# chenchen235/SemStereo

Hardware: AMD Instinct MI355X
Metric: stereo pairs/sec, hot segment (gwc+concat volumes, 3-D hourglass stack, soft-argmax), 1024x1024 maxdisp=128 (higher is better)
Workload: dtype f32; 1 GPU; BASELINE.json configs[1]: 1024x1024, maxdisp=128, batch=1/GPU x 1 GPU(s); features [B,128,H/4,W/4]+[B,256,H/8,W/8] -> disparity; input_sets_rotated=3, execution=steps round-robin on 6 HIP streams (PairPipeline); bit-identical to one stream, conv_engine=f16x3, hip_graph=False

## Files before the change

### semstereo_amd/csrc/common.cpp

```cpp
#include "common.h"

#include <stdlib.h>
#include <string.h>

#include <atomic>
#include <mutex>
#include <unordered_map>

namespace {
thread_local char g_last_error[256] = "";

int env_int(const char* name) {
    const char* v = getenv(name);
    if (v == nullptr) return -1;
    return ((v[0] >= '0' && v[0] <= '9') || (v[0] == '-' && v[1] >= '0' && v[1] <= '9')) ? atoi(v) : 1;
}

ss::Tuning read_tuning() {
    ss::Tuning t;
    t.conv_tile = env_int("SS_CONV_TILE");
    t.conv_s2_mt1 = env_int("SS_CONV_S2_MT1");
    t.gwc_stream = env_int("SS_GWC_STREAM");
    t.warp_stream = env_int("SS_WARP_STREAM");
    t.warp_vec4 = env_int("SS_WARP_VEC") == 4 ? 1 : 0;
    t.warp_generic = env_int("SS_WARP_GENERIC");
    t.deconv_split = env_int("SS_DECONV_SPLIT");
    t.deconv_groups = env_int("SS_DECONV_GROUPS");
    if (t.deconv_groups > 2) t.deconv_groups = -1;
    t.deconv_stream = env_int("SS_DECONV_STREAM");
    t.wgrad_coop = env_int("SS_WGRAD_COOP");
    t.fill_hint = env_int("SS_FILL_HINT");
    return t;
}

ss::Tuning g_tuning[2];
std::atomic<int> g_tuning_slot{-1};
std::mutex g_mutex;
std::atomic<int> g_fill_hint{1};
constexpr int kMaxFillHint = 64;
std::unordered_map<unsigned long long, int> g_lds_set;
}

namespace ss {
void note_hip_error(hipError_t e) {
    const char* s = hipGetErrorString(e);
    strncpy(g_last_error, s ? s : "unknown hip error", sizeof(g_last_error) - 1);
    g_last_error[sizeof(g_last_error) - 1] = 0;
}

const Tuning& tuning() {
    int slot = g_tuning_slot.load(std::memory_order_acquire);
    if (slot < 0) {
        std::lock_guard<std::mutex> lock(g_mutex);
        slot = g_tuning_slot.load(std::memory_order_relaxed);
        if (slot < 0) {
            g_tuning[0] = read_tuning();
            g_tuning_slot.store(slot = 0, std::memory_order_release);
        }
    }
    return g_tuning[slot];
}

int fill_hint() {
    const int env = tuning().fill_hint;
    const int h = env >= 1 ? env : g_fill_hint.load(std::memory_order_relaxed);
    return h < 1 ? 1 : (h > kMaxFillHint ? kMaxFillHint : h);
}

int ensure_dynamic_lds(const void* kernel, int bytes) {
    if (bytes <= 64 * 1024) return SS_OK;
    int dev = 0;
    if (hipGetDevice(&dev) != hipSuccess) dev = 0;
    const unsigned long long key = (unsigned long long)reinterpret_cast<uintptr_t>(kernel) * 64ull + (unsigned)dev;
    std::lock_guard<std::mutex> lock(g_mutex);
    auto it = g_lds_set.find(key);
    if (it != g_lds_set.end() && it->second >= bytes) return SS_OK;
    hipError_t e = hipFuncSetAttribute(kernel, hipFuncAttributeMaxDynamicSharedMemorySize, bytes);
    if (e != hipSuccess) {
        note_hip_error(e);
        return SS_ERR_LAUNCH;
    }
    g_lds_set[key] = bytes;
    return SS_OK;
}

int resident_workgroups(const void* kernel, int block, int lds_bytes) {
    static std::unordered_map<unsigned long long, int> cache;
    int dev = 0;
    if (hipGetDevice(&dev) != hipSuccess) dev = 0;
    const unsigned long long key = (unsigned long long)reinterpret_cast<uintptr_t>(kernel) * 64ull + (unsigned)dev;
    std::lock_guard<std::mutex> lock(g_mutex);
    auto it = cache.find(key);
    if (it != cache.end()) return it->second;
    int per_cu = 0, cus = 0;
    if (hipOccupancyMaxActiveBlocksPerMultiprocessor(&per_cu, kernel, block, (size_t)lds_bytes) != hipSuccess || per_cu < 1) per_cu = 2;
    if (hipDeviceGetAttribute(&cus, hipDeviceAttributeMultiprocessorCount, dev) != hipSuccess || cus < 1) cus = 256;
    (void)hipGetLastError();
    return cache[key] = per_cu * cus;
}
}

extern "C" int ss_reload_tuning(void) {
    std::lock_guard<std::mutex> lock(g_mutex);
    const int cur = g_tuning_slot.load(std::memory_order_relaxed);
    const int nxt = cur == 0 ? 1 : 0;
    g_tuning[nxt] = read_tuning();
    g_tuning_slot.store(nxt, std::memory_order_release);
    return SS_OK;
}

extern "C" int ss_set_fill_hint(int pairs_in_flight) {
    return g_fill_hint.exchange(pairs_in_flight < 1 ? 1 : (pairs_in_flight > kMaxFillHint ? kMaxFillHint : pairs_in_flight), std::memory_order_relaxed);
}

extern "C" int ss_get_fill_hint(void) { return ss::fill_hint(); }

extern "C" int ss_abi_version(void) { return 20; }

extern "C" const char* ss_status_string(int status) {
    switch (status) {
        case SS_OK: return "ok";
        case SS_ERR_INVALID: return "invalid argument (null pointer, non-positive size, or C % groups != 0)";
        case SS_ERR_UNSUPPORTED: return "shape not supported by the gfx950 kernels";
        case SS_ERR_LAUNCH: return "kernel launch failed (see ss_last_hip_error)";
        default: return "unknown status";
    }
}

extern "C" const char* ss_last_hip_error(void) { return g_last_error; }
```

### semstereo_amd/csrc/common.h

```cpp
#pragma once
#include <hip/hip_runtime.h>
#include <stdint.h>

#include "../../include/semstereo_hip.h"

namespace ss {

constexpr int kWave = 64;

void note_hip_error(hipError_t e);

inline int check_launch() {
    hipError_t e = hipGetLastError();
    if (e != hipSuccess) {
        note_hip_error(e);
        return SS_ERR_LAUNCH;
    }
    return SS_OK;
}

inline hipStream_t as_stream(ss_stream_t s) { return reinterpret_cast<hipStream_t>(s); }

struct Tuning {
    int conv_tile;
    int conv_s2_mt1;
    int gwc_stream;
    int warp_stream;
    int warp_vec4;
    int warp_generic;
    int deconv_split;
    int deconv_groups;
    int deconv_stream;
    int wgrad_coop;
    int fill_hint;
};
const Tuning& tuning();
int fill_hint();

int ensure_dynamic_lds(const void* kernel, int bytes);
int resident_workgroups(const void* kernel, int block, int lds_bytes);

__host__ __device__ inline int ceil_div(int a, int b) { return (a + b - 1) / b; }

inline int range_halo(int dmin, int ndisp) {
    const int a = -dmin, b = dmin + ndisp - 1;
    const int m = a > b ? a : b;
    return m <= 0 ? 0 : (m + 3) / 4 * 4;
}
__host__ __device__ inline long long ceil_div_ll(long long a, long long b) { return (a + b - 1) / b; }

struct Packed {
    long long terms, total;
};
inline float* scales_of(void* wsplit, const Packed& p) { return reinterpret_cast<float*>(static_cast<char*>(wsplit) + p.terms); }
inline const float* scales_of(const void* wsplit, const Packed& p) {
    return reinterpret_cast<const float*>(static_cast<const char*>(wsplit) + p.terms);
}

__device__ __forceinline__ float mul_rn(float a, float b) {
#pragma clang fp contract(off)
    return a * b;
}
__device__ __forceinline__ float add_rn(float a, float b) {
#pragma clang fp contract(off)
    return a + b;
}
__device__ __forceinline__ float sub_rn(float a, float b) {
#pragma clang fp contract(off)
    return a - b;
}
__device__ __forceinline__ float exp_fast(float x) {
    const float L = 1.44269502162933349609375f, Llo = 1.925962991126617e-8f;
    const float t = __fmul_rn(x, L);
    const float e = __fmaf_rn(x, L, -t) + x * Llo;
    const float p = __builtin_amdgcn_exp2f(t);
    return __fmaf_rn(p, e * 0.693147180559945f, p);
}

__device__ __forceinline__ void lds_add(float* p, float v) {
    typedef float __attribute__((address_space(3))) * lds_ptr_t;
    __hip_atomic_fetch_add((lds_ptr_t)(p), v, __ATOMIC_RELAXED, __HIP_MEMORY_SCOPE_WORKGROUP);
}

typedef volatile float __attribute__((address_space(3))) * lds_vf_t;
typedef volatile int __attribute__((address_space(3))) * lds_vi_t;
__device__ __forceinline__ void lds_owned_add(int* tag, unsigned k, bool take, float* row, float v) {
    const int me = (int)__lane_id();
    bool pending = take;
    while (__builtin_amdgcn_ballot_w64(pending) != 0) {
        if (pending) {
            ((lds_vi_t)tag)[k] = me;
            const int won = ((lds_vi_t)tag)[k];
            const float a = ((lds_vf_t)row)[k];
            if (won == me) {
                ((lds_vf_t)row)[k] = a + v;
                pending = false;
            }
        }
    }
}
__device__ __forceinline__ void lds_owned_add2(int* tag, unsigned k, bool take, float* row_a, float va, float* row_b, float vb, bool two) {
    const int me = (int)__lane_id();
    bool pending = take;
    while (__builtin_amdgcn_ballot_w64(pending) != 0) {
        if (pending) {
            ((lds_vi_t)tag)[k] = me;
            const int won = ((lds_vi_t)tag)[k];
            const float a = ((lds_vf_t)row_a)[k];
            const float b = two ? ((lds_vf_t)row_b)[k] : 0.f;
            if (won == me) {
                ((lds_vf_t)row_a)[k] = a + va;
                if (two) ((lds_vf_t)row_b)[k] = b + vb;
                pending = false;
            }
        }
    }
}
template <int N>
__device__ __forceinline__ void lds_owned_addn(int* tag, unsigned k, bool take, float* row0, int stride, const float (&v)[N], int nlive) {
    const int me = (int)__lane_id();
    bool pending = take;
    if (nlive == N) {
        while (__builtin_amdgcn_ballot_w64(pending) != 0) {
            if (pending) {
                ((lds_vi_t)tag)[k] = me;
                const int won = ((lds_vi_t)tag)[k];
                float a[N];
#pragma unroll
                for (int n = 0; n < N; ++n) a[n] = ((lds_vf_t)(row0 + n * stride))[k];
                if (won == me) {
#pragma unroll
                    for (int n = 0; n < N; ++n) ((lds_vf_t)(row0 + n * stride))[k] = a[n] + v[n];
                    pending = false;
                }
            }
        }
        return;
    }
    while (__builtin_amdgcn_ballot_w64(pending) != 0) {
        if (pending) {
            ((lds_vi_t)tag)[k] = me;
            const int won = ((lds_vi_t)tag)[k];
            float a[N];
#pragma unroll
            for (int n = 0; n < N; ++n) a[n] = (n < nlive) ? ((lds_vf_t)(row0 + n * stride))[k] : 0.f;
            if (won == me) {
#pragma unroll
                for (int n = 0; n < N; ++n)
                    if (n < nlive) ((lds_vf_t)(row0 + n * stride))[k] = a[n] + v[n];
                pending = false;
            }
        }
    }
}
__device__ __forceinline__ float lds_ld(const float* p) { return *(const float __attribute__((address_space(3)))*)p; }
__device__ __forceinline__ float lds_get(const float* p) { return *(lds_vf_t)p; }
__device__ __forceinline__ void lds_put(float* p, float v) { *(lds_vf_t)p = v; }

typedef float lds_v4f __attribute__((ext_vector_type(4)));
__device__ __forceinline__ void lds_read16(const float* p, float* dst) {
    typedef const volatile lds_v4f __attribute__((address_space(3))) * ptr_t;
    const lds_v4f q = *(ptr_t)(p);
    dst[0] = q.x; dst[1] = q.y; dst[2] = q.z; dst[3] = q.w;
}

}

int ss_softmax_regress_split_launch(const float* logits, float* prob, float* disp, float* var, int B, int dmin, int ndisp,
                                    int H, int W, hipStream_t st);

#define SS_REQUIRE(cond)              \
    do {                                \
        if (!(cond)) return SS_ERR_INVALID; \
    } while (0)
```

### semstereo_amd/csrc/window_attention.hip

```cpp
#include <algorithm>

#include "common.h"
#include "split_f16.h"

namespace {


constexpr int HD = 8;
constexpr int HG = 4;

template <int T, int C>
struct ACfg {
    static constexpr int NTL = (T + 31) / 32;
    static constexpr int TP = NTL * 32;
    static constexpr int XS = C * TP;
    static constexpr int QKV = 3 * 32 * TP;
    static constexpr int YG = 32 * TP;
    static constexpr int FLAGS = TP;
    static constexpr int WL = C * 96;
    static constexpr size_t LDS_BYTES = (size_t)(XS + QKV + YG + FLAGS + WL) * 4;
};

template <int T, int C>
__device__ __forceinline__ void stage_window_tokens(float* __restrict__ xs, const float* __restrict__ xb, int tid, int wd, int wh,
                                                    int ww, int H, int W, int bd, int bh, int bw, size_t plane, size_t vol) {
    using A = ACfg<T, C>;
    if (bw == 4 && (W & 3) == 0 && ((reinterpret_cast<uintptr_t>(xb) & 15) == 0)) {
        constexpr int NQ = C * (A::TP / 4) / 256;
        static_assert(C * (A::TP / 4) % 256 == 0, "whole batches");
#pragma unroll
        for (int i = 0; i < NQ; ++i) {
            const int e = tid + 256 * i;
            const int tq = e % (A::TP / 4), c = e / (A::TP / 4);
            const int ih = tq % bh, id = tq / bh;
            const int gh = wh * bh + ih, gd = wd * bd + id, gw = ww * 4;
            const bool ok = gh < H && gw < W;
            const float4 q = *reinterpret_cast<const float4*>(xb + (size_t)c * vol + (size_t)gd * plane +
                                                              (size_t)min(gh, H - 1) * W + min(gw, W - 4));
            *reinterpret_cast<float4*>(&xs[e * 4]) = ok ? q : make_float4(0.f, 0.f, 0.f, 0.f);
        }
    } else {
        for (int e = tid; e < C * A::TP; e += 256) {
            const int t = e % A::TP, c = e / A::TP;
            float v = 0.f;
            if (t < T) {
                const int iw = t % bw, ih = (t / bw) % bh, id = t / (bw * bh);
                const int gw = ww * bw + iw, gh = wh * bh + ih, gd = wd * bd + id;
                if (gh < H && gw < W) v = xb[(size_t)c * vol + (size_t)gd * plane + (size_t)gh * W + gw];
            }
            xs[e] = v;
        }
    }
}

template <int T, int C>
__global__ __launch_bounds__(256) void window_attention_kernel(
    const float* __restrict__ x, const float* __restrict__ wqkv_t, const float* __restrict__ bqkv,
    const float* __restrict__ wout_t, const float* __restrict__ bout, float* __restrict__ out, int D, int H, int W,
    int bd, int bh, int bw, int nwh, int nww, int use_mask) {
    using A = ACfg<T, C>;
    extern __shared__ __attribute__((aligned(16))) float lds[];
    float* xs = lds;
    float* qkv = xs + A::XS;
    float* yg = qkv + A::QKV;
    float* flag = yg + A::YG;
    float* wl = flag + A::FLAGS;

    const int tid = threadIdx.x, lane = tid & 63, wave = tid >> 6;
    const int l31 = lane & 31, half = lane >> 5;
    int wi = blockIdx.x;
    const int ww = wi % nww; wi /= nww;
    const int wh = wi % nwh; wi /= nwh;
    const int wd = wi;
    const int b = blockIdx.y;
    const size_t plane = (size_t)H * W, vol = (size_t)D * plane;
    const float* xb = x + (size_t)b * C * vol;

    stage_window_tokens<T, C>(xs, xb, tid, wd, wh, ww, H, W, bd, bh, bw, plane, vol);
    for (int t = tid; t < A::TP; t += 256) {
        float f = 0.f;
        if (t < T) {
            const int iw = t % bw, ih = (t / bw) % bh;
            f = ((wh * bh + ih >= H) || (ww * bw + iw >= W)) ? 1.f : 0.f;
        }
        flag[t] = f;
    }
    __syncthreads();

    static_assert(C == 128, "4 waves x 32 output channels");
    f32x16 oacc[A::NTL];
#pragma unroll
    for (int n = 0; n < A::NTL; ++n)
#pragma unroll
        for (int r = 0; r < 16; ++r) oacc[n][r] = 0.f;

    const float scale = 0.35355339059327379f;
    constexpr int NGROUPS = C / (HG * HD);

    constexpr int NWQ = C * 24 / 256;
    float4 wreg[NWQ];
    const float* wsrc[NWQ];
#pragma unroll
    for (int i = 0; i < NWQ; ++i) {
        const int e = tid + 256 * i;
        wsrc[i] = wqkv_t + (size_t)(e / 24) * 3 * C + ((e % 24) / 8) * C + ((e % 24) % 8) * 4;
        wreg[i] = *reinterpret_cast<const float4*>(wsrc[i]);
    }

    for (int g = 0; g < NGROUPS; ++g) {
#pragma unroll
        for (int i = 0; i < NWQ; ++i) {
            const int e = tid + 256 * i;
            *reinterpret_cast<float4*>(&wl[(e / 24) * 96 + (e % 24) * 4]) = wreg[i];
        }
        __syncthreads();
        if (g + 1 < NGROUPS) {
#pragma unroll
            for (int i = 0; i < NWQ; ++i) wreg[i] = *reinterpret_cast<const float4*>(wsrc[i] + (g + 1) * 32);
        }
        for (int u = wave; u < 3 * A::NTL; u += 4) {
            const int mt = u / A::NTL, nt = u % A::NTL;
            const int f0 = mt * C + g * 32;
            f32x16 acc;
#pragma unroll
            for (int r = 0; r < 16; ++r) acc[r] = 0.f;
            const float* ap = wl + half * 96 + mt * 32 + l31;
            const float* bp = xs + half * A::TP + nt * 32 + l31;
#pragma unroll 8
            for (int kk = 0; kk < C; kk += 2)
                acc = __builtin_amdgcn_mfma_f32_32x32x2f32(ap[kk * 96], bp[kk * A::TP], acc, 0, 0, 0);
#pragma unroll
            for (int r = 0; r < 16; ++r) {
                const int row = (r & 3) + 8 * (r >> 2) + 4 * half;
                qkv[(mt * 32 + row) * A::TP + nt * 32 + l31] = ss::add_rn(acc[r], bqkv[f0 + row]);
            }
        }
        __syncthreads();

        static_assert(A::TP == T, "windows of 64 / 96 tokens are whole 32-token tiles");
        for (int u = wave; u < HG * A::NTL; u += 4) {
            const int hh = u / A::NTL, qt = u % A::NTL;
            f32x16 st[A::NTL];
#pragma unroll
            for (int kt = 0; kt < A::NTL; ++kt) {
#pragma unroll
                for (int r = 0; r < 16; ++r) st[kt][r] = 0.f;
#pragma unroll
                for (int sd = 0; sd < HD / 2; ++sd)
                    st[kt] = __builtin_amdgcn_mfma_f32_32x32x2f32(
                        qkv[(32 + hh * HD + 2 * sd + half) * A::TP + kt * 32 + l31],
                        qkv[(hh * HD + 2 * sd + half) * A::TP + qt * 32 + l31],
                        st[kt], 0, 0, 0);
            }
            const float fq = flag[qt * 32 + l31];
            float mx = -INFINITY;
#pragma unroll
            for (int kt = 0; kt < A::NTL; ++kt)
#pragma unroll
                for (int r = 0; r < 16; ++r) {
                    float d = ss::mul_rn(st[kt][r], scale);
                    if (use_mask && flag[kt * 32 + (r & 3) + 8 * (r >> 2) + 4 * half] != fq) d = ss::add_rn(d, -1000.0f);
                    st[kt][r] = d;
                    mx = fmaxf(mx, d);
                }
            mx = fmaxf(mx, __shfl_xor(mx, 32));
            float sum = 0.f;
#pragma unroll
            for (int kt = 0; kt < A::NTL; ++kt)
#pragma unroll
                for (int r = 0; r < 16; ++r) { st[kt][r] = ss::exp_fast(st[kt][r] - mx); sum = ss::add_rn(sum, st[kt][r]); }
            sum = ss::add_rn(sum, __shfl_xor(sum, 32));
            const float rsum = 1.0f / sum;
            f32x16 ot;
#pragma unroll
            for (int r = 0; r < 16; ++r) ot[r] = 0.f;
            const float* vrow = qkv + (64 + hh * HD + (l31 & 7)) * A::TP + 4 * half;
#pragma unroll
            for (int kt = 0; kt < A::NTL; ++kt)
#pragma unroll
                for (int r = 0; r < 16; ++r) {
                    const float vv = (l31 < HD) ? vrow[kt * 32 + (r & 3) + 8 * (r >> 2)] : 0.f;
                    ot = __builtin_amdgcn_mfma_f32_32x32x2f32(vv, ss::mul_rn(st[kt][r], rsum), ot, 0, 0, 0);
                }
#pragma unroll
            for (int r = 0; r < 4; ++r) yg[(hh * HD + 4 * half + r) * A::TP + qt * 32 + l31] = ot[r];
        }
        __syncthreads();

        {
            const float* ap = wout_t + (size_t)(g * 32 + half) * C + wave * 32 + l31;
            const float* bp = yg + half * A::TP + l31;
#pragma unroll
            for (int kk = 0; kk < 32; kk += 2) {
                const float a = ap[(size_t)kk * C];
#pragma unroll
                for (int n = 0; n < A::NTL; ++n)
                    oacc[n] = __builtin_amdgcn_mfma_f32_32x32x2f32(a, bp[kk * A::TP + n * 32], oacc[n], 0, 0, 0);
            }
        }
        __syncthreads();
    }

    float* ob = out + (size_t)b * C * vol;
#pragma unroll
    for (int n = 0; n < A::NTL; ++n) {
        const int t = n * 32 + l31;
        if (t >= T) continue;
        const int iw = t % bw, ih = (t / bw) % bh, id = t / (bw * bh);
        const int gw = ww * bw + iw, gh = wh * bh + ih, gd = wd * bd + id;
        if (gh >= H || gw >= W) continue;
        const size_t pos = (size_t)gd * plane + (size_t)gh * W + gw;
#pragma unroll
        for (int r = 0; r < 16; ++r) {
            const int co = wave * 32 + (r & 3) + 8 * (r >> 2) + 4 * half;
            ob[(size_t)co * vol + pos] = ss::add_rn(oacc[n][r], bout[co]);
        }
    }
}

template <int T, int C>
__device__ __forceinline__ void attend_head_group(float* __restrict__ qkv, const float* __restrict__ flag, const unsigned (&vmax_w)[4],
                                                  float* __restrict__ y, int b, int g, int wd, int wh, int ww, int D, int H, int W,
                                                  int bd, int bh, int bw, int use_mask);

template <int T, int C>
__global__ __launch_bounds__(256) void window_attention_core(const float* __restrict__ qkv_in, const float* __restrict__ bqkv,
                                                              float* __restrict__ y, int D, int H, int W, int bd, int bh,
                                                              int bw, int nwh, int nww, int use_mask) {
    using A = ACfg<T, C>;
    static_assert(A::TP == T, "windows of 64 / 96 tokens are whole 32-token tiles");
    __shared__ __attribute__((aligned(16))) float qkv[3 * 32 * A::TP];
    __shared__ float flag[A::TP];
    const int tid = threadIdx.x, lane = tid & 63, wave = tid >> 6;
    constexpr int NGROUPS = C / (HG * HD);
    int wi = blockIdx.x;
    const int g = wi % NGROUPS; wi /= NGROUPS;
    const int ww = wi % nww; wi /= nww;
    const int wh = wi % nwh; wi /= nwh;
    const int wd = wi;
    const int b = blockIdx.y;
    const size_t plane = (size_t)H * W, vol = (size_t)D * plane;
    const float* qb = qkv_in + (size_t)b * 3 * C * vol;

    __shared__ unsigned vmax_w[4];
    float vm = 0.f;
    if (bw == 4 && (W & 3) == 0 && ((reinterpret_cast<uintptr_t>(qkv_in) & 15) == 0)) {
        constexpr int NQ = 96 * (A::TP / 4) / 256;
        static_assert(96 * (A::TP / 4) % 256 == 0, "whole batches");
#pragma unroll
        for (int i = 0; i < NQ; ++i) {
            const int e = tid + 256 * i;
            const int tq = e % (A::TP / 4), row = e / (A::TP / 4);
            const int f = (row >> 5) * C + g * 32 + (row & 31);
            const int ih = tq % bh, id = tq / bh;
            const int gh = wh * bh + ih, gd = wd * bd + id, gw = ww * 4;
            const bool ok = gh < H && gw < W;
            const float4 q = *reinterpret_cast<const float4*>(qb + (size_t)f * vol + (size_t)gd * plane +
                                                              (size_t)min(gh, H - 1) * W + min(gw, W - 4));
            const float bf = bqkv[f];
            const float4 v4 = ok ? q : make_float4(bf, bf, bf, bf);
            *reinterpret_cast<float4*>(&qkv[e * 4]) = v4;
            if (row >= 64) vm = fmaxf(vm, fmaxf(fmaxf(fabsf(v4.x), fabsf(v4.y)), fmaxf(fabsf(v4.z), fabsf(v4.w))));
        }
    } else {
        for (int e = tid; e < 96 * A::TP; e += 256) {
            const int t = e % A::TP, row = e / A::TP;
            const int f = (row >> 5) * C + g * 32 + (row & 31);
            const int iw = t % bw, ih = (t / bw) % bh, id = t / (bw * bh);
            const int gw = ww * bw + iw, gh = wh * bh + ih, gd = wd * bd + id;
            const float v1 = (gh < H && gw < W) ? qb[(size_t)f * vol + (size_t)gd * plane + (size_t)gh * W + gw] : bqkv[f];
            qkv[e] = v1;
            if (row >= 64) vm = fmaxf(vm, fabsf(v1));
        }
    }
    {
        const unsigned wm = wave_max_bits(__float_as_uint(vm));
        if (lane == 0) vmax_w[wave] = wm;
    }
    for (int t = tid; t < A::TP; t += 256) {
        const int iw = t % bw, ih = (t / bw) % bh;
        flag[t] = ((wh * bh + ih >= H) || (ww * bw + iw >= W)) ? 1.f : 0.f;
    }
    __syncthreads();
    attend_head_group<T, C>(qkv, flag, vmax_w, y, b, g, wd, wh, ww, D, H, W, bd, bh, bw, use_mask);
}

template <int T, int C>
__device__ __forceinline__ void attend_head_group(float* __restrict__ qkv, const float* __restrict__ flag, const unsigned (&vmax_w)[4],
                                                  float* __restrict__ y, int b, int g, int wd, int wh, int ww, int D, int H, int W,
                                                  int bd, int bh, int bw, int use_mask) {
    using A = ACfg<T, C>;
    const int tid = threadIdx.x, lane = tid & 63, wave = tid >> 6;
    const int l31 = lane & 31, half = lane >> 5;
    const size_t plane = (size_t)H * W, vol = (size_t)D * plane;
    const float scale = 0.35355339059327379f;
    const int e_v = workgroup_exponent(vmax_w);
    const float v_scale = scale_for(e_v);
    const float pv_unscale = unscale_for(e_v) * (1.0f / 16384.0f);
    for (int wk = tid; wk < 32 * (A::TP / 16); wk += 256) {
        float* base = qkv + (64 + wk / (A::TP / 16)) * A::TP + (wk % (A::TP / 16)) * 16;
        float f[16];
#pragma unroll
        for (int k4 = 0; k4 < 4; ++k4) ss::lds_read16(base + 4 * k4, &f[4 * k4]);
#pragma unroll
        for (int h = 0; h < 2; ++h) {
            unsigned hi[4], lo[4];
#pragma unroll
            for (int j = 0; j < 4; ++j) {
                const int t0 = (j < 2) ? 4 * h + 2 * j : 8 + 4 * h + 2 * (j - 2);
                split2_pk_f16(f[t0] * v_scale, f[t0 + 1] * v_scale, hi[j], lo[j]);
            }
            *reinterpret_cast<uint4*>(base + 8 * h) = make_uint4(hi[0], hi[1], hi[2], hi[3]);
            *reinterpret_cast<uint4*>(base + 8 * h + 4) = make_uint4(lo[0], lo[1], lo[2], lo[3]);
        }
    }
    __syncthreads();
    float* yb = y + (size_t)b * C * vol;
    for (int u = wave; u < HG * A::NTL; u += 4) {
        const int hh = u / A::NTL, qt = u % A::NTL;
        f32x16 st[A::NTL];
#pragma unroll
        for (int kt = 0; kt < A::NTL; ++kt) {
#pragma unroll
            for (int r = 0; r < 16; ++r) st[kt][r] = 0.f;
#pragma unroll
            for (int sd = 0; sd < HD / 2; ++sd)
                st[kt] = __builtin_amdgcn_mfma_f32_32x32x2f32(
                    qkv[(32 + hh * HD + 2 * sd + half) * A::TP + kt * 32 + l31],
                    qkv[(hh * HD + 2 * sd + half) * A::TP + qt * 32 + l31],
                    st[kt], 0, 0, 0);
        }
        const float fq = flag[qt * 32 + l31];
        float mx = -INFINITY;
#pragma unroll
        for (int kt = 0; kt < A::NTL; ++kt)
#pragma unroll
            for (int r = 0; r < 16; ++r) {
                float d = ss::mul_rn(st[kt][r], scale);
                if (use_mask && flag[kt * 32 + (r & 3) + 8 * (r >> 2) + 4 * half] != fq) d = ss::add_rn(d, -1000.0f);
                st[kt][r] = d;
                mx = fmaxf(mx, d);
            }
        mx = fmaxf(mx, __shfl_xor(mx, 32));
        float sum = 0.f;
#pragma unroll
        for (int kt = 0; kt < A::NTL; ++kt)
#pragma unroll
            for (int r = 0; r < 16; ++r) { st[kt][r] = ss::exp_fast(st[kt][r] - mx); sum = ss::add_rn(sum, st[kt][r]); }
        sum = ss::add_rn(sum, __shfl_xor(sum, 32));
        const float rsum = 1.0f / sum;
        f32x16 ot;
#pragma unroll
        for (int r = 0; r < 16; ++r) ot[r] = 0.f;
        const float* vrow = qkv + (64 + hh * HD + (l31 & 7)) * A::TP + 8 * half;
        const float ps = rsum * 16384.0f;
#pragma unroll
        for (int kt = 0; kt < A::NTL; ++kt)
#pragma unroll
            for (int s8 = 0; s8 < 2; ++s8) {
                float vh[4], vl[4];
                ss::lds_read16(vrow + kt * 32 + 16 * s8, vh);
                ss::lds_read16(vrow + kt * 32 + 16 * s8 + 4, vl);
                unsigned bh_[4], bl_[4];
#pragma unroll
                for (int j = 0; j < 4; ++j)
                    split2_pk_f16(st[kt][8 * s8 + 2 * j] * ps, st[kt][8 * s8 + 2 * j + 1] * ps, bh_[j], bl_[j]);
                const f16x8 a_hi = __builtin_bit_cast(f16x8, make_float4(vh[0], vh[1], vh[2], vh[3]));
                const f16x8 a_lo = __builtin_bit_cast(f16x8, make_float4(vl[0], vl[1], vl[2], vl[3]));
                const f16x8 b_hi = __builtin_bit_cast(f16x8, make_uint4(bh_[0], bh_[1], bh_[2], bh_[3]));
                const f16x8 b_lo = __builtin_bit_cast(f16x8, make_uint4(bl_[0], bl_[1], bl_[2], bl_[3]));
                ot = __builtin_amdgcn_mfma_f32_32x32x16_f16(a_hi, b_lo, ot, 0, 0, 0);
                ot = __builtin_amdgcn_mfma_f32_32x32x16_f16(a_lo, b_hi, ot, 0, 0, 0);
                ot = __builtin_amdgcn_mfma_f32_32x32x16_f16(a_hi, b_hi, ot, 0, 0, 0);
            }
#pragma unroll
        for (int r = 0; r < 4; ++r) ot[r] *= pv_unscale;
        const int t = qt * 32 + l31;
        const int iw = t % bw, ih = (t / bw) % bh, id = t / (bw * bh);
        const int gw = ww * bw + iw, gh = wh * bh + ih, gd = wd * bd + id;
        if (gh < H && gw < W) {
            const size_t pos = (size_t)gd * plane + (size_t)gh * W + gw;
#pragma unroll
            for (int r = 0; r < 4; ++r) yb[(size_t)(g * 32 + hh * HD + 4 * half + r) * vol + pos] = ot[r];
        }
    }
}

template <int T, int C, int NTERMS, int KH>
__global__ __launch_bounds__(256, KH == 2 ? 4 : 3) void window_attention_proj(const float* __restrict__ x, const uint4* __restrict__ wsplit,
                                                              const float* __restrict__ bqkv, float* __restrict__ y, int D, int H,
                                                              int W, int bd, int bh, int bw, int nwh, int nww, int use_mask) {
    using A = ACfg<T, C>;
    static_assert(A::TP == T && C % (32 * KH) == 0 && (KH == 1 || KH == 2), "whole 32-token tiles, whole K-steps per stage");
    constexpr int NC = (NTERMS == 6) ? 3 : 2;
    constexpr int KS = C / 16;
    constexpr int CH = C / KH;
    __shared__ __attribute__((aligned(16))) float buf[(CH > 96 ? CH : 96) * A::TP];
    __shared__ float flag[A::TP];
    __shared__ unsigned vmax_w[4];
    const int tid = threadIdx.x, lane = tid & 63, wave = tid >> 6;
    const int l31 = lane & 31, half = lane >> 5;
    constexpr int NGROUPS = C / (HG * HD);
    int wi = blockIdx.x;
    const int g = wi % NGROUPS; wi /= NGROUPS;
    const int ww = wi % nww; wi /= nww;
    const int wh = wi % nwh; wi /= nwh;
    const int wd = wi;
    const int b = blockIdx.y;
    const size_t plane = (size_t)H * W, vol = (size_t)D * plane;

    for (int t = tid; t < A::TP; t += 256) {
        const int iw = t % bw, ih = (t / bw) % bh;
        flag[t] = ((wh * bh + ih >= H) || (ww * bw + iw >= W)) ? 1.f : 0.f;
    }
    constexpr int NU = (3 * A::NTL + 3) / 4;
    f32x16 acc[NU];
#pragma unroll
    for (int i = 0; i < NU; ++i)
#pragma unroll
        for (int r = 0; r < 16; ++r) acc[i][r] = 0.f;
#pragma unroll
    for (int kh = 0; kh < KH; ++kh) {
        if (kh > 0) __syncthreads();
        stage_window_tokens<T, CH>(buf, x + ((size_t)b * C + kh * CH) * vol, tid, wd, wh, ww, H, W, bd, bh, bw, plane, vol);
        __syncthreads();
#pragma unroll
        for (int i = 0; i < NU; ++i) {
            const int u = wave + 4 * i;
            if (u >= 3 * A::NTL) continue;
            const int mt = u / A::NTL, nt = u % A::NTL;
            const uint4* ap = wsplit + (size_t)(mt * (C / 32) + g) * KS * 3 * 64 + half * 32 + l31;
            const float* bp = buf + 8 * half * A::TP + nt * 32 + l31;
#pragma unroll
            for (int k = 0; k < KS / KH; ++k) {
                const int ks = kh * (KS / KH) + k;
                bf16x8 a[NC];
#pragma unroll
                for (int c = 0; c < NC; ++c) a[c] = __builtin_bit_cast(bf16x8, ap[(ks * 3 + c) * 64]);
                unsigned bh_[4], bm_[4], bl_[4];
#pragma unroll
                for (int j = 0; j < 4; ++j)
                    split3_pk(bp[(k * 16 + 2 * j) * A::TP], bp[(k * 16 + 2 * j + 1) * A::TP], bh_[j], bm_[j], bl_[j]);
                const bf16x8 h8 = __builtin_bit_cast(bf16x8, make_uint4(bh_[0], bh_[1], bh_[2], bh_[3]));
                const bf16x8 m8 = __builtin_bit_cast(bf16x8, make_uint4(bm_[0], bm_[1], bm_[2], bm_[3]));
                if (NTERMS == 6) {
                    const bf16x8 l8 = __builtin_bit_cast(bf16x8, make_uint4(bl_[0], bl_[1], bl_[2], bl_[3]));
                    acc[i] = __builtin_amdgcn_mfma_f32_32x32x16_bf16(a[1], m8, acc[i], 0, 0, 0);
                    acc[i] = __builtin_amdgcn_mfma_f32_32x32x16_bf16(a[0], l8, acc[i], 0, 0, 0);
                    acc[i] = __builtin_amdgcn_mfma_f32_32x32x16_bf16(a[NC - 1], h8, acc[i], 0, 0, 0);
                }
                acc[i] = __builtin_amdgcn_mfma_f32_32x32x16_bf16(a[0], m8, acc[i], 0, 0, 0);
                acc[i] = __builtin_amdgcn_mfma_f32_32x32x16_bf16(a[1], h8, acc[i], 0, 0, 0);
                acc[i] = __builtin_amdgcn_mfma_f32_32x32x16_bf16(a[0], h8, acc[i], 0, 0, 0);
            }
        }
    }
    float bias[NU][16];
#pragma unroll
    for (int i = 0; i < NU; ++i) {
        const int u = wave + 4 * i;
        if (u >= 3 * A::NTL) continue;
#pragma unroll
        for (int r = 0; r < 16; ++r) bias[i][r] = bqkv[(u / A::NTL) * C + g * 32 + (r & 3) + 8 * (r >> 2) + 4 * half];
    }
    __syncthreads();
    float vm = 0.f;
#pragma unroll
    for (int i = 0; i < NU; ++i) {
        const int u = wave + 4 * i;
        if (u >= 3 * A::NTL) continue;
        const int mt = u / A::NTL, nt = u % A::NTL;
#pragma unroll
        for (int r = 0; r < 16; ++r) {
            const float v = ss::add_rn(acc[i][r], bias[i][r]);
            buf[(mt * 32 + (r & 3) + 8 * (r >> 2) + 4 * half) * A::TP + nt * 32 + l31] = v;
            if (mt == 2) vm = fmaxf(vm, fabsf(v));
        }
    }
    {
        const unsigned wm = wave_max_bits(__float_as_uint(vm));
        if (lane == 0) vmax_w[wave] = wm;
    }
    __syncthreads();
    attend_head_group<T, C>(buf, flag, vmax_w, y, b, g, wd, wh, ww, D, H, W, bd, bh, bw, use_mask);
}

#ifndef SS_ATTN_PROJ_KH96
#define SS_ATTN_PROJ_KH96 2
#endif
template <int T, int NTERMS>
int launch_attn_proj(const float* x, const void* wsplit, const float* bqkv, float* y, int B, int D, int H, int W, int bd, int bh,
                     int bw, hipStream_t st) {
    const int nwd = D / bd, nwh = ss::ceil_div(H, bh), nww = ss::ceil_div(W, bw);
    const int use_mask = (H % bh != 0) && (W % bw != 0);
    const long long nblk = (long long)nwd * nwh * nww * (128 / (HG * HD));
    if (nblk > 0x7fffffffLL || B > 65535) return SS_ERR_UNSUPPORTED;
    hipLaunchKernelGGL((window_attention_proj<T, 128, NTERMS, T == 96 ? SS_ATTN_PROJ_KH96 : 1>), dim3((unsigned)nblk, B), dim3(256), 0, st, x,
                       reinterpret_cast<const uint4*>(wsplit), bqkv, y, D, H, W, bd, bh, bw, nwh, nww, use_mask);
    return ss::check_launch();
}

template <int T>
int launch_attn_core(const float* qkv, const float* bqkv, float* y, int B, int D, int H, int W, int bd, int bh, int bw,
                     hipStream_t st) {
    const int nwd = D / bd, nwh = ss::ceil_div(H, bh), nww = ss::ceil_div(W, bw);
    const int use_mask = (H % bh != 0) && (W % bw != 0);
    const long long nblk = (long long)nwd * nwh * nww * (128 / (HG * HD));
    if (nblk > 0x7fffffffLL || B > 65535) return SS_ERR_UNSUPPORTED;
    hipLaunchKernelGGL((window_attention_core<T, 128>), dim3((unsigned)nblk, B), dim3(256), 0, st, qkv, bqkv, y, D, H, W, bd,
                       bh, bw, nwh, nww, use_mask);
    return ss::check_launch();
}

template <int T>
int launch_attn(const float* x, const float* wqkv_t, const float* bqkv, const float* wout_t, const float* bout,
                float* out, int B, int D, int H, int W, int bd, int bh, int bw, hipStream_t st) {
    using A = ACfg<T, 128>;
    const int nwd = D / bd, nwh = ss::ceil_div(H, bh), nww = ss::ceil_div(W, bw);
    const int use_mask = (H % bh != 0) && (W % bw != 0);
    auto kern = window_attention_kernel<T, 128>;
    if (A::LDS_BYTES > 64 * 1024) {
        if (ss::ensure_dynamic_lds(reinterpret_cast<const void*>(kern), (int)A::LDS_BYTES) != SS_OK) return SS_ERR_LAUNCH;
    }
    const long long nwin = (long long)nwd * nwh * nww;
    if (nwin > 0x7fffffffLL || B > 65535) return SS_ERR_UNSUPPORTED;
    hipLaunchKernelGGL(kern, dim3((unsigned)nwin, B), dim3(256), A::LDS_BYTES, st, x, wqkv_t, bqkv, wout_t, bout, out, D,
                       H, W, bd, bh, bw, nwh, nww, use_mask);
    return ss::check_launch();
}

}

extern "C" int ss_window_attention_fwd(const float* x, const float* wqkv_t, const float* bqkv, const float* wout_t,
                                       const float* bout, float* out, int B, int C, int D, int H, int W, int heads,
                                       int bd, int bh, int bw, ss_stream_t stream) {
    SS_REQUIRE(x && wqkv_t && bqkv && wout_t && bout && out);
    SS_REQUIRE(B > 0 && C > 0 && D > 0 && H > 0 && W > 0 && heads > 0 && bd > 0 && bh > 0 && bw > 0);
    SS_REQUIRE(D % bd == 0);
    if (C != 128 || heads != 16) return SS_ERR_UNSUPPORTED;
    const int T = bd * bh * bw;
    hipStream_t st = ss::as_stream(stream);
    if (T == 64) return launch_attn<64>(x, wqkv_t, bqkv, wout_t, bout, out, B, D, H, W, bd, bh, bw, st);
    if (T == 96) return launch_attn<96>(x, wqkv_t, bqkv, wout_t, bout, out, B, D, H, W, bd, bh, bw, st);
    return SS_ERR_UNSUPPORTED;
}

extern "C" int ss_window_attention_core_fwd(const float* qkv, const float* bqkv, float* y, int B, int C, int D, int H,
                                            int W, int heads, int bd, int bh, int bw, ss_stream_t stream) {
    SS_REQUIRE(qkv && bqkv && y);
    SS_REQUIRE(B > 0 && C > 0 && D > 0 && H > 0 && W > 0 && heads > 0 && bd > 0 && bh > 0 && bw > 0);
    SS_REQUIRE(D % bd == 0);
    if (C != 128 || heads != 16) return SS_ERR_UNSUPPORTED;
    const int T = bd * bh * bw;
    hipStream_t st = ss::as_stream(stream);
    if (T == 64) return launch_attn_core<64>(qkv, bqkv, y, B, D, H, W, bd, bh, bw, st);
    if (T == 96) return launch_attn_core<96>(qkv, bqkv, y, B, D, H, W, bd, bh, bw, st);
    return SS_ERR_UNSUPPORTED;
}

extern "C" int ss_window_attention_proj_fwd(const float* x, const void* wqkv_split, const float* bqkv, float* y, int B, int C,
                                            int D, int H, int W, int heads, int bd, int bh, int bw, int nterms,
                                            ss_stream_t stream) {
    SS_REQUIRE(x && wqkv_split && bqkv && y);
    SS_REQUIRE(B > 0 && C > 0 && D > 0 && H > 0 && W > 0 && heads > 0 && bd > 0 && bh > 0 && bw > 0);
    SS_REQUIRE(D % bd == 0 && (nterms == 3 || nterms == 6));
    SS_REQUIRE((reinterpret_cast<uintptr_t>(wqkv_split) & 15) == 0);
    if (C != 128 || heads != 16) return SS_ERR_UNSUPPORTED;
    const int T = bd * bh * bw;
    hipStream_t st = ss::as_stream(stream);
#define SS_AP(TV)                                                                                                     \
    if (T == TV)                                                                                                      \
        return nterms == 6 ? launch_attn_proj<TV, 6>(x, wqkv_split, bqkv, y, B, D, H, W, bd, bh, bw, st)              \
                           : launch_attn_proj<TV, 3>(x, wqkv_split, bqkv, y, B, D, H, W, bd, bh, bw, st);
    SS_AP(64)
    SS_AP(96)
#undef SS_AP
    return SS_ERR_UNSUPPORTED;
}
```

Before: 651.7 pairs/s.

## Pre-split window tokens into bf16 terms once when staging attention projection

Adds a staging path that converts each window's fp32 tokens into packed bf16 high/mid/low split terms once, storing them in swizzled LDS. The projection MFMA loop then loads them directly, so the split is no longer recomputed in every wave that reuses the same tokens. A vectorized float4 load path covers bw==4, and attend_head_group gets a compile-time mask specialization. It is on by default for T==96 with KH=2 and can be toggled with SS_ATTN_SPLIT_ONCE. The cost is larger LDS use (NC/2 times the rows), which may lower occupancy.

```diff
diff --git a/semstereo_amd/csrc/common.cpp b/semstereo_amd/csrc/common.cpp
--- a/semstereo_amd/csrc/common.cpp
+++ b/semstereo_amd/csrc/common.cpp
@@ -30,6 +30,7 @@
     t.deconv_stream = env_int("SS_DECONV_STREAM");
     t.wgrad_coop = env_int("SS_WGRAD_COOP");
     t.fill_hint = env_int("SS_FILL_HINT");
+    t.attn_split_once = env_int("SS_ATTN_SPLIT_ONCE");
     return t;
 }
 
diff --git a/semstereo_amd/csrc/common.h b/semstereo_amd/csrc/common.h
--- a/semstereo_amd/csrc/common.h
+++ b/semstereo_amd/csrc/common.h
@@ -33,6 +33,7 @@
     int deconv_stream;
     int wgrad_coop;
     int fill_hint;
+    int attn_split_once;
 };
 const Tuning& tuning();
 int fill_hint();
diff --git a/semstereo_amd/csrc/window_attention.hip b/semstereo_amd/csrc/window_attention.hip
--- a/semstereo_amd/csrc/window_attention.hip
+++ b/semstereo_amd/csrc/window_attention.hip
@@ -49,6 +49,64 @@
                 if (gh < H && gw < W) v = xb[(size_t)c * vol + (size_t)gd * plane + (size_t)gh * W + gw];
             }
             xs[e] = v;
+        }
+    }
+}
+
+template <int T, int CH, int NTS>
+__device__ __forceinline__ void stage_window_tokens_split(uint4* __restrict__ xt, const float* __restrict__ xb, int tid, int wd, int wh,
+                                                          int ww, int H, int W, int bd, int bh, int bw, size_t plane, size_t vol) {
+    using A = ACfg<T, CH>;
+    static_assert(CH % 16 == 0 && A::TP % 8 == 0 && (NTS == 2 || NTS == 3), "whole K-steps, whole swizzle groups");
+    auto put = [&](const float (&v)[8], int cg, int t) {
+        unsigned h[4], m[4], l[4];
+#pragma unroll
+        for (int j = 0; j < 4; ++j) split3_pk(v[2 * j], v[2 * j + 1], h[j], m[j], l[j]);
+        uint4* dst = xt + ((cg >> 1) * NTS * 2 + (cg & 1)) * A::TP + (t ^ ((t >> 3) & 3));
+        dst[0] = make_uint4(h[0], h[1], h[2], h[3]);
+        dst[2 * A::TP] = make_uint4(m[0], m[1], m[2], m[3]);
+        if (NTS == 3) dst[4 * A::TP] = make_uint4(l[0], l[1], l[2], l[3]);
+    };
+    if (bw == 4 && (W & 3) == 0 && ((reinterpret_cast<uintptr_t>(xb) & 15) == 0)) {
+        constexpr int TQ = A::TP / 4, NI = (CH / 8) * TQ;
+        static_assert(NI <= 256, "one pass");
+        if (tid < NI) {
+            const int tq = tid % TQ, cg = tid / TQ;
+            const int ih = tq % bh, id = tq / bh;
+            const int gh = wh * bh + ih, gd = wd * bd + id, gw = ww * 4;
+            const bool ok = gh < H && gw < W;
+            const float* src = xb + (size_t)(cg * 8) * vol + (size_t)gd * plane + (size_t)min(gh, H - 1) * W + min(gw, W - 4);
+            float4 q[8];
+#pragma unroll
+            for (int j = 0; j < 8; ++j) {
+                const float4 v4 = *reinterpret_cast<const float4*>(src + (size_t)j * vol);
+                q[j] = ok ? v4 : make_float4(0.f, 0.f, 0.f, 0.f);
+            }
+            float v[8];
+#pragma unroll
+            for (int j = 0; j < 8; ++j) v[j] = q[j].x;
+            put(v, cg, 4 * tq);
+#pragma unroll
+            for (int j = 0; j < 8; ++j) v[j] = q[j].y;
+            put(v, cg, 4 * tq + 1);
+#pragma unroll
+            for (int j = 0; j < 8; ++j) v[j] = q[j].z;
+            put(v, cg, 4 * tq + 2);
+#pragma unroll
+            for (int j = 0; j < 8; ++j) v[j] = q[j].w;
+            put(v, cg, 4 * tq + 3);
+        }
+    } else {
+        for (int e = tid; e < (CH / 8) * A::TP; e += 256) {
+            const int t = e % A::TP, cg = e / A::TP;
+            const int iw = t % bw, ih = (t / bw) % bh, id = t / (bw * bh);
+            const int gw = ww * bw + iw, gh = wh * bh + ih, gd = wd * bd + id;
+            const bool ok = t < T && gh < H && gw < W;
+            float v[8];
+#pragma unroll
+            for (int j = 0; j < 8; ++j)
+                v[j] = ok ? xb[(size_t)(cg * 8 + j) * vol + (size_t)gd * plane + (size_t)gh * W + gw] : 0.f;
+            put(v, cg, t);
         }
     }
 }
@@ -218,7 +276,7 @@
     }
 }
 
-template <int T, int C>
+template <int T, int C, int MASK = -1>
 __device__ __forceinline__ void attend_head_group(float* __restrict__ qkv, const float* __restrict__ flag, const unsigned (&vmax_w)[4],
                                                   float* __restrict__ y, int b, int g, int wd, int wh, int ww, int D, int H, int W,
                                                   int bd, int bh, int bw, int use_mask);
@@ -285,7 +343,7 @@
     attend_head_group<T, C>(qkv, flag, vmax_w, y, b, g, wd, wh, ww, D, H, W, bd, bh, bw, use_mask);
 }
 
-template <int T, int C>
+template <int T, int C, int MASK>
 __device__ __forceinline__ void attend_head_group(float* __restrict__ qkv, const float* __restrict__ flag, const unsigned (&vmax_w)[4],
                                                   float* __restrict__ y, int b, int g, int wd, int wh, int ww, int D, int H, int W,
                                                   int bd, int bh, int bw, int use_mask) {
@@ -330,14 +388,16 @@
                     qkv[(hh * HD + 2 * sd + half) * A::TP + qt * 32 + l31],
                     st[kt], 0, 0, 0);
         }
-        const float fq = flag[qt * 32 + l31];
+        const bool masked = MASK < 0 ? use_mask != 0 : MASK != 0;
+        const float fq = MASK == 0 ? 0.f : flag[qt * 32 + l31];
         float mx = -INFINITY;
 #pragma unroll
         for (int kt = 0; kt < A::NTL; ++kt)
 #pragma unroll
             for (int r = 0; r < 16; ++r) {
                 float d = ss::mul_rn(st[kt][r], scale);
-                if (use_mask && flag[kt * 32 + (r & 3) + 8 * (r >> 2) + 4 * half] != fq) d = ss::add_rn(d, -1000.0f);
+                const float* fk = &flag[kt * 32 + (r & 3) + 8 * (r >> 2) + 4 * half];
+                if (masked && (MASK == 1 ? lds_read4(fk) : *fk) != fq) d = ss::add_rn(d, -1000.0f);
                 st[kt][r] = d;
                 mx = fmaxf(mx, d);
             }
@@ -386,7 +446,7 @@
     }
 }
 
-template <int T, int C, int NTERMS, int KH>
+template <int T, int C, int NTERMS, int KH, bool ONCE>
 __global__ __launch_bounds__(256, KH == 2 ? 4 : 3) void window_attention_proj(const float* __restrict__ x, const uint4* __restrict__ wsplit,
                                                               const float* __restrict__ bqkv, float* __restrict__ y, int D, int H,
                                                               int W, int bd, int bh, int bw, int nwh, int nww, int use_mask) {
@@ -395,7 +455,8 @@
     constexpr int NC = (NTERMS == 6) ? 3 : 2;
     constexpr int KS = C / 16;
     constexpr int CH = C / KH;
-    __shared__ __attribute__((aligned(16))) float buf[(CH > 96 ? CH : 96) * A::TP];
+    constexpr int XROWS = ONCE ? CH * NC / 2 : CH;
+    __shared__ __attribute__((aligned(16))) float buf[(XROWS > 96 ? XROWS : 96) * A::TP];
     __shared__ float flag[A::TP];
     __shared__ unsigned vmax_w[4];
     const int tid = threadIdx.x, lane = tid & 63, wave = tid >> 6;
@@ -422,7 +483,9 @@
 #pragma unroll
     for (int kh = 0; kh < KH; ++kh) {
         if (kh > 0) __syncthreads();
-        stage_window_tokens<T, CH>(buf, x + ((size_t)b * C + kh * CH) * vol, tid, wd, wh, ww, H, W, bd, bh, bw, plane, vol);
+        const float* xs = x + ((size_t)b * C + kh * CH) * vol;
+        if constexpr (ONCE) stage_window_tokens_split<T, CH, NC>(reinterpret_cast<uint4*>(buf), xs, tid, wd, wh, ww, H, W, bd, bh, bw, plane, vol);
+        else stage_window_tokens<T, CH>(buf, xs, tid, wd, wh, ww, H, W, bd, bh, bw, plane, vol);
         __syncthreads();
 #pragma unroll
         for (int i = 0; i < NU; ++i) {
@@ -431,6 +494,7 @@
             const int mt = u / A::NTL, nt = u % A::NTL;
             const uint4* ap = wsplit + (size_t)(mt * (C / 32) + g) * KS * 3 * 64 + half * 32 + l31;
             const float* bp = buf + 8 * half * A::TP + nt * 32 + l31;
+            const uint4* bs = reinterpret_cast<const uint4*>(buf) + half * A::TP + nt * 32 + (l31 ^ ((l31 >> 3) & 3));
 #pragma unroll
             for (int k = 0; k < KS / KH; ++k) {
                 const int ks = kh * (KS / KH) + k;
@@ -438,13 +502,20 @@
 #pragma unroll
                 for (int c = 0; c < NC; ++c) a[c] = __builtin_bit_cast(bf16x8, ap[(ks * 3 + c) * 64]);
                 unsigned bh_[4], bm_[4], bl_[4];
-#pragma unroll
-                for (int j = 0; j < 4; ++j)
-                    split3_pk(bp[(k * 16 + 2 * j) * A::TP], bp[(k * 16 + 2 * j + 1) * A::TP], bh_[j], bm_[j], bl_[j]);
-                const bf16x8 h8 = __builtin_bit_cast(bf16x8, make_uint4(bh_[0], bh_[1], bh_[2], bh_[3]));
-                const bf16x8 m8 = __builtin_bit_cast(bf16x8, make_uint4(bm_[0], bm_[1], bm_[2], bm_[3]));
+                bf16x8 h8, m8, l8;
+                if constexpr (ONCE) {
+                    h8 = __builtin_bit_cast(bf16x8, bs[(k * NC + 0) * 2 * A::TP]);
+                    m8 = __builtin_bit_cast(bf16x8, bs[(k * NC + 1) * 2 * A::TP]);
+                    if (NTERMS == 6) l8 = __builtin_bit_cast(bf16x8, bs[(k * NC + NC - 1) * 2 * A::TP]);
+                } else {
+#pragma unroll
+                    for (int j = 0; j < 4; ++j)
+                        split3_pk(bp[(k * 16 + 2 * j) * A::TP], bp[(k * 16 + 2 * j + 1) * A::TP], bh_[j], bm_[j], bl_[j]);
+                    h8 = __builtin_bit_cast(bf16x8, make_uint4(bh_[0], bh_[1], bh_[2], bh_[3]));
+                    m8 = __builtin_bit_cast(bf16x8, make_uint4(bm_[0], bm_[1], bm_[2], bm_[3]));
+                    if (NTERMS == 6) l8 = __builtin_bit_cast(bf16x8, make_uint4(bl_[0], bl_[1], bl_[2], bl_[3]));
+                }
                 if (NTERMS == 6) {
-                    const bf16x8 l8 = __builtin_bit_cast(bf16x8, make_uint4(bl_[0], bl_[1], bl_[2], bl_[3]));
                     acc[i] = __builtin_amdgcn_mfma_f32_32x32x16_bf16(a[1], m8, acc[i], 0, 0, 0);
                     acc[i] = __builtin_amdgcn_mfma_f32_32x32x16_bf16(a[0], l8, acc[i], 0, 0, 0);
                     acc[i] = __builtin_amdgcn_mfma_f32_32x32x16_bf16(a[NC - 1], h8, acc[i], 0, 0, 0);
@@ -482,7 +553,12 @@
         if (lane == 0) vmax_w[wave] = wm;
     }
     __syncthreads();
-    attend_head_group<T, C>(buf, flag, vmax_w, y, b, g, wd, wh, ww, D, H, W, bd, bh, bw, use_mask);
+    if constexpr (ONCE) {
+        if (use_mask) attend_head_group<T, C, 1>(buf, flag, vmax_w, y, b, g, wd, wh, ww, D, H, W, bd, bh, bw, use_mask);
+        else attend_head_group<T, C, 0>(buf, flag, vmax_w, y, b, g, wd, wh, ww, D, H, W, bd, bh, bw, use_mask);
+    } else {
+        attend_head_group<T, C>(buf, flag, vmax_w, y, b, g, wd, wh, ww, D, H, W, bd, bh, bw, use_mask);
+    }
 }
 
 #ifndef SS_ATTN_PROJ_KH96
@@ -495,8 +571,13 @@
     const int use_mask = (H % bh != 0) && (W % bw != 0);
     const long long nblk = (long long)nwd * nwh * nww * (128 / (HG * HD));
     if (nblk > 0x7fffffffLL || B > 65535) return SS_ERR_UNSUPPORTED;
-    hipLaunchKernelGGL((window_attention_proj<T, 128, NTERMS, T == 96 ? SS_ATTN_PROJ_KH96 : 1>), dim3((unsigned)nblk, B), dim3(256), 0, st, x,
-                       reinterpret_cast<const uint4*>(wsplit), bqkv, y, D, H, W, bd, bh, bw, nwh, nww, use_mask);
+    const int once_env = ss::tuning().attn_split_once;
+    if (once_env >= 0 ? once_env != 0 : T == 96)
+        hipLaunchKernelGGL((window_attention_proj<T, 128, NTERMS, 2, true>), dim3((unsigned)nblk, B), dim3(256), 0, st, x,
+                           reinterpret_cast<const uint4*>(wsplit), bqkv, y, D, H, W, bd, bh, bw, nwh, nww, use_mask);
+    else
+        hipLaunchKernelGGL((window_attention_proj<T, 128, NTERMS, T == 96 ? SS_ATTN_PROJ_KH96 : 1, false>), dim3((unsigned)nblk, B), dim3(256), 0, st, x,
+                           reinterpret_cast<const uint4*>(wsplit), bqkv, y, D, H, W, bd, bh, bw, nwh, nww, use_mask);
     return ss::check_launch();
 }
 
```

Result: no change. 651.6 pairs/s (median of 2 runs) (-0.0%).
